# tomneda/DABstar

Hardware: NVIDIA B200
Metric: Mode I DAB frames/s decoded (IQ->Viterbi) (higher is better)
Workload: dtype f32

## Files before the change

### dabstar_b200/csrc/engine.cu

```cuda
#include "../../include/dabstar_b200.h"
#include "kernels.h"
#include "tables.h"
#include "hostpool.h"
#include "fft2048.cuh"

#include <algorithm>
#include <array>
#include <atomic>
#include <chrono>
#include <climits>
#include <cmath>
#include <cstdint>
#include <cstdarg>
#include <cstdio>
#include <cstring>
#include <map>
#include <memory>
#include <string>
#include <vector>

using namespace dab;

namespace
{
// ... 252 lines not shown
  }
  ctx->h_bin_signed.resize(K_CARR);
  host_freq_interleaver(ctx->h_bin_signed.data());
  ctx->h_prs.resize(T_U);
  host_phase_table(ctx->h_prs.data());
  std::vector<float2> w(T_U);
  host_w2048(w.data());
  std::vector<int16_t> bin_idx(K_CARR), rel(K_CARR);
  for (int k = 0; k < K_CARR; k++)
  {
    const int b = ctx->h_bin_signed[k];
    bin_idx[k] = (int16_t)(b < 0 ? b + T_U : b);
    rel[k] = (int16_t)(b < 0 ? b + K_CARR / 2 : b + K_CARR / 2 - 1);
  }
  std::vector<uint8_t> prbs(PRBS_LEN);
  host_prbs(prbs.data(), PRBS_LEN);
  bool ok = true;
  ok = ok && cudaMalloc(&ctx->tab.w2048, sizeof(float2) * T_U) == cudaSuccess;
  ok = ok && cudaMalloc(&ctx->tab.prs, sizeof(float2) * T_U) == cudaSuccess;
  ok = ok && cudaMalloc(&ctx->tab.ref_arg_conj, sizeof(float2) * T_U) == cudaSuccess;
  ok = ok && cudaMalloc(&ctx->tab.bin_of_k, sizeof(int16_t) * K_CARR) == cudaSuccess;
  ok = ok && cudaMalloc(&ctx->tab.rel_of_k, sizeof(int16_t) * K_CARR) == cudaSuccess;
  ok = ok && cudaMalloc(&ctx->tab.prbs, PRBS_LEN) == cudaSuccess;
  std::vector<uint16_t> slot_w(16 * FFT_THREADS), slot_r(K_CARR);
  host_fft_epilogue_layout(bin_idx.data(), slot_w.data(), slot_r.data());
  ok = ok && cudaMalloc(&ctx->tab.fft_slot_w, sizeof(uint16_t) * slot_w.size()) == cudaSuccess;
  ok = ok && cudaMalloc(&ctx->tab.fft_slot_r, sizeof(uint16_t) * slot_r.size()) == cudaSuccess;
  ok = ok && cudaMemcpy(ctx->tab.fft_slot_w, slot_w.data(), sizeof(uint16_t) * slot_w.size(), cudaMemcpyHostToDevice) == cudaSuccess;
  ok = ok && cudaMemcpy(ctx->tab.fft_slot_r, slot_r.data(), sizeof(uint16_t) * slot_r.size(), cudaMemcpyHostToDevice) == cudaSuccess;
  ok = ok && cudaMemcpy(ctx->tab.w2048, w.data(), sizeof(float2) * T_U, cudaMemcpyHostToDevice) == cudaSuccess;
  ok = ok && cudaMemcpy(ctx->tab.prs, ctx->h_prs.data(), sizeof(float2) * T_U, cudaMemcpyHostToDevice) == cudaSuccess;
  ok = ok && cudaMemcpy(ctx->tab.bin_of_k, bin_idx.data(), sizeof(int16_t) * K_CARR, cudaMemcpyHostToDevice) == cudaSuccess;
  ok = ok && cudaMemcpy(ctx->tab.rel_of_k, rel.data(), sizeof(int16_t) * K_CARR, cudaMemcpyHostToDevice) == cudaSuccess;
  ok = ok && cudaMemcpy(ctx->tab.prbs, prbs.data(), PRBS_LEN, cudaMemcpyHostToDevice) == cudaSuccess;
  ok = ok && launch_init_ref_arg(ctx->stream, ctx->tab, &ctx->launches) == cudaSuccess;
  ok = ok && cudaStreamSynchronize(ctx->stream) == cudaSuccess;
  if (!ok) { dabstar_destroy(ctx.release()); return DABSTAR_E_CUDA; }
  push_profile(ctx.get(), make_fic_profile());
  *out = ctx.release();
  return DABSTAR_OK;
}

extern "C" void dabstar_destroy(dabstar_ctx * ctx)
{
  if (!ctx) return;
  cudaSetDevice(ctx->device);
  cudaFree(ctx->tab.w2048); cudaFree(ctx->tab.prs); cudaFree(ctx->tab.ref_arg_conj);
  cudaFree(ctx->tab.bin_of_k); cudaFree(ctx->tab.rel_of_k); cudaFree(ctx->tab.prbs); cudaFree(ctx->tab.fft_slot_w); cudaFree(ctx->tab.fft_slot_r);
// ... 2580 lines not shown
```

### dabstar_b200/csrc/ofdm_kernels.cu

```cuda
#include "fft2048.cuh"
#include "kernels.h"
#include "devcache.h"

#include <algorithm>
#include <cstdlib>
#include <type_traits>

namespace dab
{
namespace
{
template <int FMT> struct Raw;
template <> struct Raw<FMT_U8> { typedef unsigned short type; typedef unsigned reg; };
template <> struct Raw<FMT_I16> { typedef short2 type; typedef short2 reg; };
template <> struct Raw<FMT_CF32> { typedef float2 type; typedef float2 reg; };

__device__ __forceinline__ float2 to_cf(unsigned v)
{
  const float2 m = make_float2(__uint_as_float(__byte_perm(v, 0x4B000000u, 0x7540)), __uint_as_float(__byte_perm(v, 0x4B000000u, 0x7541)));
  const float2 f = __fadd2_rn(m, make_float2(-8388608.0f, -8388608.0f));
  return __ffma2_rn(f, make_float2(1.0f / 128.0f, 1.0f / 128.0f), make_float2(-127.38f / 128.0f, -127.38f / 128.0f));
}
__device__ __forceinline__ float2 to_cf(short2 v) { return __fmul2_rn(make_float2((float)v.x, (float)v.y), make_float2(1.0f / 32768.0f, 1.0f / 32768.0f)); }
__device__ __forceinline__ float2 to_cf(float2 v) { return v; }
// ... 121 lines not shown
__device__ __forceinline__ void bulk_g2s(unsigned dst, const void * src, unsigned bytes, unsigned bar)
{
  asm volatile("cp.async.bulk.shared::cluster.global.mbarrier::complete_tx::bytes [%0], [%1], %2, [%3];" ::"r"(dst), "l"(src), "r"(bytes), "r"(bar) : "memory");
}
__device__ __forceinline__ void mbar_wait(unsigned bar, unsigned parity)
{
  unsigned ok;
  do
  {
    asm volatile("{\n\t.reg .pred p;\n\tmbarrier.try_wait.parity.shared::cta.b64 p, [%1], %2;\n\tselp.u32 %0, 1, 0, p;\n\t}" : "=r"(ok) : "r"(bar), "r"(parity) : "memory");
  } while (!ok);
}

template <int FMT>
__device__ __forceinline__ bool item_async(const SymbolItem & it) { return it.out >= 0 && it.start >= 8 && it.start + T_U + 8 <= it.n_total; }

__device__ __forceinline__ int mod_fs32(int x)
{
  const int r = x % FS;
  return r < 0 ? r + FS : r;
}

template <int FMT>
__device__ __forceinline__ void convert_mix(float2 (&v)[16], const typename Raw<FMT>::reg (&r)[16], int f, int ph, const float2 * step, int tid)
{
#pragma unroll
  for (int n1 = 0; n1 < 16; n1++) v[n1] = to_cf(r[n1]);
  if (f == 0)
  {
    if (ph == 0) return;
    const float2 c = step[0];
#pragma unroll
    for (int n1 = 0; n1 < 16; n1++) v[n1] = cmul(v[n1], c);
    return;
  }
  const float2 s0 = osc(mod_fs32(ph - f * (tid + 1)));
#pragma unroll
  for (int n1 = 0; n1 < 16; n1++) v[n1] = cmul(v[n1], n1 == 0 ? s0 : cmul(s0, step[n1]));
}

template <int FMT>
__global__ void __launch_bounds__(FFT_THREADS, 5) k_fft_frames(const FrameDesc * __restrict__ frames, int n_items, const RecInput * __restrict__ recs,
                                                               const float2 * __restrict__ w2048, const uint16_t * __restrict__ slot_w,
                                                               const uint16_t * __restrict__ slot_r, float2 * __restrict__ X)
{
  typedef typename Raw<FMT>::type T;
  extern __shared__ __align__(16) unsigned char fft_stage[];
  __shared__ __align__(16) float2 smem[FFT_SMEM_F2];
  __shared__ float2 tw2s[FFT_TW2_F2];
  __shared__ float2 step[16];
  __shared__ unsigned short pos[16 * FFT_THREADS];
  __shared__ unsigned rpos[K_CARR / 2];
  __shared__ __align__(8) unsigned long long mbar[2];
  const int tid = threadIdx.x;
  FftTwiddles tw;
  fft_load_twiddles(tw, w2048, tw2s, tid);
#pragma unroll
  for (int i = 0; i < 16; i++) pos[i * FFT_THREADS + tid] = (unsigned short)(slot_w[i * FFT_THREADS + tid] * (int)sizeof(float2));
  for (int p = tid; p < K_CARR / 2; p += FFT_THREADS)
    rpos[p] = (unsigned)slot_r[2 * p] * (unsigned)sizeof(float2) | ((unsigned)slot_r[2 * p + 1] * (unsigned)sizeof(float2)) << 16;
  static_assert(2048 <= FFT_SMEM_F2, "the staging slots (16 per write group) must fit the transform buffer");
  const unsigned stage0 = smem_addr_u32(fft_stage);
  const unsigned bar0 = smem_addr_u32(mbar);
  constexpr int SB = fft_stage_bytes<FMT>();
  if (tid == 0)
  {
    mbar_init(bar0, 1);
    mbar_init(bar0 + 8, 1);
    asm volatile("fence.mbarrier_init.release.cluster;" ::: "memory");
    asm volatile("fence.proxy.async.shared::cta;" ::: "memory");
  }
  __syncthreads();

  const int per = n_items / (int)gridDim.x, rem = n_items - per * (int)gridDim.x;
  int item = (int)blockIdx.x * per + min((int)blockIdx.x, rem);
  const int item_end = item + per + ((int)blockIdx.x < rem ? 1 : 0);
  int buf = 0, fi = item / X_ROWS, row = item - fi * X_ROWS;
  unsigned phase_bits = 0;
  FrameDesc fd;
  RecInput rin;
  SymbolItem cur;
  cur.out = -1;
  int dph = 0;
  int step_f = 0;
  int step_ph = -1;
  auto issue = [&](const SymbolItem & it, int b) {
    if (tid == 0)
    {
      const unsigned long long a = (unsigned long long)(reinterpret_cast<const T *>(it.iq) + it.start);
      mbar_expect_tx(bar0 + 8u * (unsigned)b, (unsigned)SB);
      bulk_g2s(stage0 + (unsigned)(b * SB), reinterpret_cast<const void *>(a & ~15ull), (unsigned)SB, bar0 + 8u * (unsigned)b);
    }
  };
  if (item < item_end)
  {
    fd = frames[fi];
    rin = recs[fd.rec];
    cur = symbol_item(fd, rin, row);
    dph = mod_fs32(-(int)(((long long)fd.f_data * T_S) % FS));
    if (item_async<FMT>(cur)) issue(cur, 0);
  }
  while (item < item_end)
  {
    const int next = item + 1;
    SymbolItem nxt;
    nxt.out = -1;
    if (next < item_end)
    {
      if (++row == X_ROWS)
      {
        row = 0;
        fi++;
        fd = frames[fi];
        rin = recs[fd.rec];
        dph = mod_fs32(-(int)(((long long)fd.f_data * T_S) % FS));
      }
      if (row >= 2 && row <= 75)
      {
        nxt.iq = cur.iq;
        nxt.n_total = cur.n_total;
        nxt.start = cur.start + T_S;
        nxt.f = cur.f;
        nxt.ph = cur.ph + dph;
        if (nxt.ph >= FS) nxt.ph -= FS;
        nxt.out = row > fd.n_syms ? -1 : ((long long)fd.xslot * X_ROWS + row) * K_CARR;
      }
      else nxt = symbol_item(fd, rin, row);
      if (item_async<FMT>(nxt)) issue(nxt, buf ^ 1);
    }
    if (cur.out >= 0)
    {
      float2 v[16];
      if (cur.f != 0 ? cur.f != step_f : (cur.ph != 0 && cur.ph != step_ph))
      {
        __syncthreads();
        if (cur.f != 0)
        {
          if (tid < 16) step[tid] = osc(mod_fs32(-(int)(((long long)cur.f * 128 * tid) % FS)));
          step_f = cur.f;
          step_ph = -1;
        }
        else
        {
          if (tid == 0) step[0] = osc(cur.ph);
          step_ph = cur.ph;
          step_f = 0;
        }
        __syncthreads();
      }
      if (item_async<FMT>(cur))
      {
        mbar_wait(bar0 + 8u * (unsigned)buf, (phase_bits >> buf) & 1u);
        phase_bits ^= 1u << buf;
        const unsigned off = (unsigned)((unsigned long long)(reinterpret_cast<const T *>(cur.iq) + cur.start) & 15ull);
        const T * sp = reinterpret_cast<const T *>(fft_stage + buf * SB + off) + tid;
        typename Raw<FMT>::reg r[16];
#pragma unroll
        for (int n1 = 0; n1 < 16; n1++) r[n1] = sp[128 * n1];
        convert_mix<FMT>(v, r, cur.f, cur.ph, step, tid);
      }
      else
      {
        typename Raw<FMT>::reg r[16];
        fetch_symbol<FMT>(r, cur.iq, cur.n_total, cur.start, tid);
        convert_mix<FMT>(v, r, cur.f, cur.ph, step, tid);
        if (!(cur.start >= 0 && cur.start + T_U <= cur.n_total))
        {
#pragma unroll
          for (int n1 = 0; n1 < 16; n1++)
          {
            const long long i = cur.start + 128 * n1 + tid;
            if (i < 0 || i >= cur.n_total) v[n1] = make_float2(0.0f, 0.0f);
          }
        }
      }
      fft_stage1(v, tw, smem, tid);
      __syncthreads();
      fft_stage2_read(v, smem, tid);
      __syncthreads();
      fft_stage2(v, tw, smem, tid);
      __syncthreads();
      fft_stage3(v, smem, tid);
      __syncthreads();
      unsigned char * sbase = reinterpret_cast<unsigned char *>(smem);
#pragma unroll
      for (int i = 0; i < 16; i++) *reinterpret_cast<float2 *>(sbase + pos[i * FFT_THREADS + tid]) = v[i];
      __syncthreads();
      float4 * out = reinterpret_cast<float4 *>(X + cur.out);
#pragma unroll
      for (int i = 0; i < K_CARR / 2 / FFT_THREADS; i++)
      {
        const int p = tid + FFT_THREADS * i;
        const unsigned rp = rpos[p];
        const float2 a = *reinterpret_cast<const float2 *>(sbase + (rp & 0xffffu)), b = *reinterpret_cast<const float2 *>(sbase + (rp >> 16));
        out[p] = make_float4(a.x, b.x, a.y, b.y);
      }
    }
    __syncthreads();
    cur = nxt;
    item = next;
    buf ^= 1;
  }
}

__global__ void __launch_bounds__(FFT_THREADS, 4) k_fft_batch(const float2 * __restrict__ in, float2 * __restrict__ out, int n, int sign,
                                                              const float2 * __restrict__ w2048)
{
  __shared__ float2 smem[FFT_SMEM_F2];
  __shared__ float2 tw2s[FFT_TW2_F2];
  const int tid = threadIdx.x;
  FftTwiddles tw;
  fft_load_twiddles(tw, w2048, tw2s, tid);
  __syncthreads();
  for (int item = blockIdx.x; item < n; item += gridDim.x)
  {
    float2 v[16];
#pragma unroll
    for (int n1 = 0; n1 < 16; n1++)
    {
      v[n1] = in[(size_t)item * T_U + 128 * n1 + tid];
      if (sign > 0) v[n1].y = -v[n1].y;
    }
    fft2048_to_smem(v, tw, smem, tid);
    for (int i = tid; i < T_U; i += FFT_THREADS)
    {
      float2 r = smem[fft_nat(i)];
      if (sign > 0) r.y = -r.y;
      out[(size_t)item * T_U + i] = r;
    }
    __syncthreads();
  }
}

template <int FMT>
__global__ void __launch_bounds__(FFT_THREADS, 4) k_fft_null(const FrameDesc * __restrict__ frames, int n_frames, const RecInput * __restrict__ recs,
                                                             const float2 * __restrict__ w2048, float2 * __restrict__ out)
{
  __shared__ float2 smem[FFT_SMEM_F2];
  __shared__ float2 step[16];
  __shared__ float2 tw2s[FFT_TW2_F2];
  const int tid = threadIdx.x;
  FftTwiddles tw;
  fft_load_twiddles(tw, w2048, tw2s, tid);
  __syncthreads();
  for (int fi = blockIdx.x; fi < n_frames; fi += gridDim.x)
  {
    const FrameDesc fd = frames[fi];
    const RecInput rin = recs[fd.rec];
    const SymbolItem it = symbol_item(fd, rin, X_ROWS - 1);
    float2 v[16];
    load_symbol<FMT>(v, it.iq, it.n_total, it.start, it.f, it.ph, step, tid);
    if (!(it.start >= 0 && it.start + T_U <= it.n_total))
    {
#pragma unroll
      for (int n1 = 0; n1 < 16; n1++)
      {
        const long long i = it.start + 128 * n1 + tid;
        if (i < 0 || i >= it.n_total) v[n1] = make_float2(0.0f, 0.0f);
      }
    }
    fft2048_to_smem(v, tw, smem, tid);
    for (int i = tid; i < T_U; i += FFT_THREADS) out[(size_t)fi * T_U + i] = smem[fft_nat(i)];
    __syncthreads();
  }
}

__global__ void k_reorder_frames(const float2 * __restrict__ fft_nat, int n_rows, const int16_t * __restrict__ bin_of_k, float2 * __restrict__ X)
{
  const int row = blockIdx.x;
  if (row >= n_rows) return;
  for (int p = threadIdx.x; p < K_CARR / 2; p += blockDim.x)
  {
    const float2 a = fft_nat[(size_t)row * T_U + bin_of_k[2 * p]], b = fft_nat[(size_t)row * T_U + bin_of_k[2 * p + 1]];
    reinterpret_cast<float4 *>(X + (size_t)row * K_CARR)[p] = make_float4(a.x, b.x, a.y, b.y);
  }
}

__device__ __forceinline__ float warp_sum(float v)
{
#pragma unroll
  for (int o = 16; o > 0; o >>= 1) v += __shfl_xor_sync(0xffffffffu, v, o);
  return v;
}

__device__ void prs_correlate_cta(float2 (&v)[16], const FftTwiddles & tw, const float2 * __restrict__ prs, float threshold, int strongest,
                                  float2 * smem, float * red, int * result, int tid)
// ... 1067 lines not shown
    const long long b = o >> 11;
    const int j = (int)(o & 2047);
    const long long lo = b * block_in + base[j] - shift;
    const float r = frac[j], r1 = __fsub_rn(1.0f, r);
    const float2 hi_v = lo + 1 < n_in ? in[lo + 1] : make_float2(0.f, 0.f);
    const float2 lo_v = lo >= 0 ? in[lo] : make_float2(0.f, 0.f);
    out[o] = make_float2(__fadd_rn(__fmul_rn(hi_v.x, r), __fmul_rn(lo_v.x, r1)), __fadd_rn(__fmul_rn(hi_v.y, r), __fmul_rn(lo_v.y, r1)));
  }
}

template <typename F> cudaError_t dispatch_fmt(int fmt, F && f)
{
  switch (fmt)
  {
  case FMT_CF32: f(std::integral_constant<int, FMT_CF32>()); break;
  case FMT_U8: f(std::integral_constant<int, FMT_U8>()); break;
  case FMT_I16: f(std::integral_constant<int, FMT_I16>()); break;
  default: return cudaErrorInvalidValue;
  }
  return cudaGetLastError();
}

inline int fft_grid(int n_items) { return n_items < N_SM * 4 ? n_items : N_SM * 4; }
}

cudaError_t launch_init_ref_arg(cudaStream_t s, const DeviceTables & t, unsigned long long * lc)
{
  k_init_ref_arg<<<1, FFT_THREADS, 0, s>>>(t.w2048, t.prs, t.ref_arg_conj);
  if (lc) (*lc)++;
  return cudaGetLastError();
}

cudaError_t launch_fft_batch(cudaStream_t s, const DeviceTables & t, const float2 * in, float2 * out, int n, int sign, unsigned long long * lc)
{
  if (n <= 0) return cudaSuccess;
  k_fft_batch<<<fft_grid(n), FFT_THREADS, 0, s>>>(in, out, n, sign, t.w2048);
  if (lc) (*lc)++;
  return cudaGetLastError();
}

cudaError_t launch_fft_frames(cudaStream_t s, const DeviceTables & t, const FrameDesc * frames, int n_frames, const RecInput * recs, int fmt,
                              float2 * X, int max_ctas_per_sm, unsigned long long * lc)
{
  if (n_frames <= 0) return cudaSuccess;
  const int n_items = n_frames * X_ROWS;
  if (lc) (*lc)++;
  return dispatch_fmt(fmt, [&](auto F) {
    constexpr int FMT = decltype(F)::value;
    constexpr int stage = 2 * fft_stage_bytes<FMT>();
    const LaunchProps lp = launch_props((const void *)k_fft_frames<FMT>, FFT_THREADS, stage, stage);
    int per_sm = lp.err == cudaSuccess && lp.ctas_per_sm > 0 ? lp.ctas_per_sm : 4;
    if (max_ctas_per_sm > 0) per_sm = std::min(per_sm, max_ctas_per_sm);
    k_fft_frames<FMT><<<std::min(n_items, lp.n_sm * per_sm), FFT_THREADS, stage, s>>>(frames, n_items, recs, t.w2048, t.fft_slot_w, t.fft_slot_r, X);
  });
}

cudaError_t launch_reorder_frames(cudaStream_t s, const DeviceTables & t, const float2 * fft_nat, int n_frames, float2 * X, unsigned long long * lc)
{
  if (n_frames <= 0) return cudaSuccess;
  k_reorder_frames<<<n_frames * X_ROWS, 256, 0, s>>>(fft_nat, n_frames * X_ROWS, t.bin_of_k, X);
  if (lc) (*lc)++;
  return cudaGetLastError();
}

size_t demap_ring_bytes(int n_work) { return sizeof(unsigned long long) * (size_t)std::max(n_work, 1) * DM3_RING * DM5_WARPS + 256; }
static size_t demap5_smem_bytes(int lag) { return sizeof(float4) * 2 * (size_t)(lag + 1 + DM5_PF) * DM5_T + sizeof(int) * (size_t)(lag + 1) * (DM5_T / 32); }
template <int LAG, bool QUAL> static const void * demap5_fn(int soft_bit_type)
{
  return soft_bit_type == 0 ? (const void *)k_demap5<0, LAG, QUAL> : (soft_bit_type == 1 ? (const void *)k_demap5<1, LAG, QUAL> : (const void *)k_demap5<2, LAG, QUAL>);
}
template <int LAG> static const void * demap5_fn(int soft_bit_type, bool qual) { return qual ? demap5_fn<LAG, true>(soft_bit_type) : demap5_fn<LAG, false>(soft_bit_type); }

cudaError_t launch_demap(cudaStream_t s, const DeviceTables & t, const DemapWork * work, int n_work, const FrameDesc * frames,
                         const uint8_t * null_is_tii, const float2 * X, OfdmStateDev * states, int soft_bit_type, int16_t * soft,
                         unsigned long long * ring, FrameQualSnap * qsnap, unsigned long long * lc)
{
// ... 97 lines not shown
{
  if (n <= 0) return cudaSuccess;
  k_coarse_afc_raw<<<fft_grid(n), FFT_THREADS, 0, s>>>(fft_nat, n, t.w2048, t.ref_arg_conj, offset_hz);
  if (lc) (*lc)++;
  return cudaGetLastError();
}

cudaError_t launch_ingest_convert(cudaStream_t s, const void * src, int container, int msb_first, int iq_order, float inv_scaler, const float * lut,
                                  long long n_samples, float2 * dst, unsigned long long * lc)
{
  if (n_samples <= 0) return cudaSuccess;
  const long long blocks = (n_samples + 255) / 256;
  k_ingest_convert<<<(unsigned)std::min<long long>(blocks, N_SM * 16), 256, 0, s>>>(static_cast<const unsigned char *>(src), container, msb_first, iq_order, inv_scaler, lut,
                                                                                    n_samples, dst);
  if (lc) (*lc)++;
  return cudaGetLastError();
}

cudaError_t launch_fft_null(cudaStream_t s, const DeviceTables & t, const FrameDesc * frames, int n_frames, const RecInput * recs, int fmt, float2 * out,
                            unsigned long long * lc)
{
  if (n_frames <= 0) return cudaSuccess;
  if (lc) (*lc)++;
  return dispatch_fmt(fmt, [&](auto F) { k_fft_null<decltype(F)::value><<<fft_grid(n_frames), FFT_THREADS, 0, s>>>(frames, n_frames, recs, t.w2048, out); });
}

cudaError_t launch_resample_linear(cudaStream_t s, const float2 * in, long long n_in, int block_in, int shift, const short * base, const float * frac,
                                   long long n_out, float2 * out, unsigned long long * lc)
{
  if (n_out <= 0) return cudaSuccess;
  const long long blocks = (n_out + 255) / 256;
  k_resample_linear<<<(unsigned)std::min<long long>(blocks, N_SM * 16), 256, 0, s>>>(in, n_in, block_in, shift, base, frac, n_out, out);
  if (lc) (*lc)++;
  return cudaGetLastError();
}

cudaError_t launch_dip_search(cudaStream_t s, const DipWork * work, int n, const RecInput * recs, int fmt, DipResult * out, unsigned long long * lc)
{
  if (n <= 0) return cudaSuccess;
  if (lc) (*lc)++;
  return dispatch_fmt(fmt, [&](auto F) { k_dip_search<decltype(F)::value><<<n, DIP_THREADS, 0, s>>>(work, recs, out); });
}
}
```

### dabstar_b200/csrc/tables.cu

```cuda
#include "tables.h"
#include "fft2048.cuh"
#include <vector>

#include <cmath>
#include <cstring>

namespace dab
{
static const uint32_t PI_MASK[24] = {
  0x11111113u, 0x11131113u, 0x11131313u, 0x13131313u, 0x13131333u, 0x13331333u, 0x13333333u, 0x33333333u,
  0x33333337u, 0x33373337u, 0x33373737u, 0x37373737u, 0x37373777u, 0x37773777u, 0x37777777u, 0x77777777u,
  0x7777777fu, 0x777f777fu, 0x777f7f7fu, 0x7f7f7f7fu, 0x7f7f7fffu, 0x7fff7fffu, 0x7fffffffu, 0xffffffffu };

struct UepRow { int16_t bitrate, level, L[4], PI[4]; };
static const UepRow UEP_TABLE[] = {
  {32,5, {3,4,17,0}, {5,3,2,0}}, {32,4, {3,3,18,0}, {11,6,5,0}}, {32,3, {3,4,14,3}, {15,9,6,8}},
  {32,2, {3,4,14,3}, {22,13,8,13}}, {32,1, {3,5,13,3}, {24,17,12,17}}, {48,5, {4,3,26,3}, {5,4,2,3}},
  {48,4, {3,4,26,3}, {9,6,4,6}}, {48,3, {3,4,26,3}, {15,10,6,9}}, {48,2, {3,4,26,3}, {24,14,8,15}},
  {48,1, {3,5,25,3}, {24,18,13,18}}, {56,5, {6,10,23,3}, {5,4,2,3}}, {56,4, {6,10,23,3}, {9,6,4,5}},
  {56,3, {6,12,21,3}, {16,7,6,9}}, {56,2, {6,10,23,3}, {23,13,8,13}}, {64,5, {6,9,31,2}, {5,3,2,3}},
  {64,4, {6,9,33,0}, {11,6,5,0}}, {64,3, {6,12,27,3}, {16,8,6,9}}, {64,2, {6,10,29,3}, {23,13,8,13}},
  {64,1, {6,11,28,3}, {24,18,12,18}}, {80,5, {6,10,41,3}, {6,3,2,3}}, {80,4, {6,10,41,3}, {11,6,5,6}},
  {80,3, {6,11,40,3}, {16,8,6,7}}, {80,2, {6,10,41,3}, {23,13,8,13}}, {80,1, {6,10,41,3}, {24,7,12,18}},
  {96,5, {7,9,53,3}, {5,4,2,4}}, {96,4, {7,10,52,3}, {9,6,4,6}}, {96,3, {6,12,51,3}, {16,9,6,10}},
// ... 13 lines not shown
static const int N_UEP = (int)(sizeof(UEP_TABLE) / sizeof(UEP_TABLE[0]));

static const uint8_t PRS_ROW[48] = { 0,1,2,3, 0,1,2,3, 0,1,2,3, 0,1,2,3, 0,1,2,3, 0,1,2,3,
                                     0,3,2,1, 0,3,2,1, 0,3,2,1, 0,3,2,1, 0,3,2,1, 0,3,2,1 };
static const uint8_t PRS_N[48] = { 1,2,0,1, 3,2,2,3, 2,1,2,3, 1,2,3,3, 2,2,2,1, 1,3,1,2,
                                   3,1,1,1, 2,2,1,0, 2,2,3,3, 0,2,1,3, 3,3,3,0, 3,0,1,1 };
static const uint8_t PRS_H[4][32] = {
  { 0,2,0,0,0,0,1,1,2,0,0,0,2,2,1,1, 0,2,0,0,0,0,1,1,2,0,0,0,2,2,1,1 },
  { 0,3,2,3,0,1,3,0,2,1,2,3,2,3,3,0, 0,3,2,3,0,1,3,0,2,1,2,3,2,3,3,0 },
  { 0,0,0,2,0,2,1,3,2,2,0,2,2,0,1,3, 0,0,0,2,0,2,1,3,2,2,0,2,2,0,1,3 },
  { 0,1,2,1,0,3,3,2,2,3,2,1,2,1,3,2, 0,1,2,1,0,3,3,2,2,3,2,1,2,1,3,2 } };

void host_freq_interleaver(int16_t * bin_signed)
{
  int n = 0, v = 0;
  for (int i = 0; i < T_U; i++)
  {
    if (i > 0) v = (13 * v + 511) % T_U;
    if (v == T_U / 2 || v < 256 || v > 256 + K_CARR) continue;
    bin_signed[n++] = (int16_t)(v - T_U / 2);
  }
}

void host_fft_epilogue_layout(const int16_t * bin_of_k, uint16_t * slot_w, uint16_t * slot_r)
{
  constexpr int NW = 128, NR = 96, D = 16;
  std::vector<int> carrier_of_bin(T_U, -1);
  for (int k = 0; k < K_CARR; k++) carrier_of_bin[bin_of_k[k]] = k;
  std::vector<int> wg(K_CARR, -1), rg(K_CARR, -1);
  for (int i = 0; i < 16; i++)
    for (int tid = 0; tid < FFT_THREADS; tid++)
    {
      const int c = carrier_of_bin[fft_out_index(tid, i >> 3, i & 7)];
      if (c >= 0) wg[c] = (i * 4 + (tid >> 5)) * 2 + ((tid >> 4) & 1);
    }
  for (int c = 0; c < K_CARR; c++)
  {
    const int p = c >> 1, b = c & 1, it = p / FFT_THREADS, tid = p % FFT_THREADS;
    rg[c] = ((it * 2 + b) * 4 + (tid >> 5)) * 2 + ((tid >> 4) & 1);
  }
  std::vector<int> at_w(NW * D, -1), at_r(NR * D, -1), colour(K_CARR, -1);
  for (int e = 0; e < K_CARR; e++)
  {
    const int u = wg[e], v = rg[e];
    int a = 0, b = 0;
    while (at_w[u * D + a] >= 0) a++;
    while (at_r[v * D + b] >= 0) b++;
    if (a != b)
    {
      std::vector<int> path;
      int x = v, side = 1, want = a;
      while (true)
      {
        const int f = side ? at_r[x * D + want] : at_w[x * D + want];
        if (f < 0) break;
        path.push_back(f);
        x = side ? wg[f] : rg[f];
        side ^= 1;
        want = want == a ? b : a;
      }
      for (int f : path) { at_w[wg[f] * D + colour[f]] = -1; at_r[rg[f] * D + colour[f]] = -1; }
      for (int f : path) { colour[f] = colour[f] == a ? b : a; }
      for (int f : path) { at_w[wg[f] * D + colour[f]] = f; at_r[rg[f] * D + colour[f]] = f; }
    }
    colour[e] = a;
    at_w[u * D + a] = e;
    at_r[v * D + a] = e;
  }
  for (int c = 0; c < K_CARR; c++) slot_r[c] = (uint16_t)(wg[c] * D + colour[c]);
  for (int i = 0; i < 16; i++)
    for (int tid = 0; tid < FFT_THREADS; tid++)
    {
      const int g = (i * 4 + (tid >> 5)) * 2 + ((tid >> 4) & 1);
      const int c = carrier_of_bin[fft_out_index(tid, i >> 3, i & 7)];
      if (c >= 0) { slot_w[i * FFT_THREADS + tid] = slot_r[c]; continue; }
      int a = 0;
      while (at_w[g * D + a] >= 0) a++;
      at_w[g * D + a] = K_CARR;
      slot_w[i * FFT_THREADS + tid] = (uint16_t)(g * D + a);
    }
}

void host_phase_table(float2 * prs)
{
  const float pi_2 = (float)(M_PI / 2.0);
  memset(prs, 0, sizeof(float2) * T_U);
  for (int k = -K_CARR / 2; k <= K_CARR / 2; k++)
  {
    if (k == 0) continue;
    const int blk = k < 0 ? (k + 768) / 32 : 24 + (k - 1) / 32;
    const int kmin = k < 0 ? -768 + 32 * blk : 1 + 32 * (blk - 24);
    const float phi = pi_2 * (float)(PRS_H[PRS_ROW[blk]][k - kmin] + PRS_N[blk]);
    prs[k < 0 ? k + T_U : k] = make_float2(cosf(phi), sinf(phi));
  }
}

void host_prbs(uint8_t * out, int n)
{
  unsigned reg = 0x1ff;
  for (int i = 0; i < n; i++)
  {
    const unsigned b = ((reg >> 8) ^ (reg >> 4)) & 1u;
    reg = ((reg << 1) | b) & 0x1ff;
// ... 111 lines not shown
```

### dabstar_b200/csrc/tables.h

```cpp
#pragma once
#include "common.cuh"
#include "viterbi.cuh"

namespace dab
{
void host_freq_interleaver(int16_t * bin_signed);
void host_phase_table(float2 * prs);
void host_prbs(uint8_t * out, int n);
void host_w2048(float2 * w);
void host_fft_epilogue_layout(const int16_t * bin_of_k, uint16_t * slot_w , uint16_t * slot_r );
VitProfile make_fic_profile();
VitProfile make_identity_profile(int n_bits);
bool make_msc_profile(int short_form, int bit_rate, int prot_level, VitProfile & p);
int profile_addresses(const VitProfile & p, int32_t * addr, int cap);
}
```

Before: 792,800.

## Move 2048-point FFT to one warp per symbol with warp-local epilogue

Replaces the 128-thread block-cooperative 2048-point FFT with a per-warp FFT: each lane holds 64 points, runs a radix-64 then radix-32 decomposition with a single padded shared-memory transpose, and synchronises with __syncwarp instead of __syncthreads. Work is split across warps with per-warp TMA staging buffers and mbarriers, and the bank-conflict-free carrier scatter layout is recomputed for the warp output order. The aim is to remove block-wide barriers and improve independent progress per warp. In exchange it adds heavy register pressure (64 complex values per thread plus raw inputs), uses more shared memory per warp, and runs one CTA per SM, which may lower occupancy.

```diff
diff --git a/dabstar_b200/csrc/engine.cu b/dabstar_b200/csrc/engine.cu
--- a/dabstar_b200/csrc/engine.cu
+++ b/dabstar_b200/csrc/engine.cu
@@ -298,8 +298,8 @@
   ok = ok && cudaMalloc(&ctx->tab.bin_of_k, sizeof(int16_t) * K_CARR) == cudaSuccess;
   ok = ok && cudaMalloc(&ctx->tab.rel_of_k, sizeof(int16_t) * K_CARR) == cudaSuccess;
   ok = ok && cudaMalloc(&ctx->tab.prbs, PRBS_LEN) == cudaSuccess;
-  std::vector<uint16_t> slot_w(16 * FFT_THREADS), slot_r(K_CARR);
-  host_fft_epilogue_layout(bin_idx.data(), slot_w.data(), slot_r.data());
+  std::vector<uint16_t> slot_w(T_U), slot_r(K_CARR);
+  host_fft_warp_epilogue_layout(bin_idx.data(), slot_w.data(), slot_r.data());
   ok = ok && cudaMalloc(&ctx->tab.fft_slot_w, sizeof(uint16_t) * slot_w.size()) == cudaSuccess;
   ok = ok && cudaMalloc(&ctx->tab.fft_slot_r, sizeof(uint16_t) * slot_r.size()) == cudaSuccess;
   ok = ok && cudaMemcpy(ctx->tab.fft_slot_w, slot_w.data(), sizeof(uint16_t) * slot_w.size(), cudaMemcpyHostToDevice) == cudaSuccess;
diff --git a/dabstar_b200/csrc/fft2048_warp.cuh b/dabstar_b200/csrc/fft2048_warp.cuh
--- /dev/null
+++ b/dabstar_b200/csrc/fft2048_warp.cuh
@@ -0,0 +1,134 @@
+#pragma once
+#include "fft2048.cuh"
+
+namespace dab
+{
+constexpr int FFTW_E_STRIDE = 33;
+constexpr int FFTW_E_F2 = 64 * FFTW_E_STRIDE;
+constexpr int FFTW_TW_F2 = 64 * 32;
+
+__host__ __device__ inline void fftw_load_twiddles(const float2 * w2048, float2 * tw, int tid, int nthreads)
+{
+  for (int i = tid; i < FFTW_TW_F2; i += nthreads) tw[i] = w2048[((i & 31) * (i >> 5)) & 2047];
+}
+
+__host__ __device__ constexpr float cos64(int r)
+{
+  switch (r)
+  {
+  case 0: return 1.0f;
+  case 1: return 0.99518472667219688624f;
+  case 2: return 0.98078528040323044913f;
+  case 3: return 0.95694033573220886494f;
+  case 4: return 0.92387953251128675613f;
+  case 5: return 0.88192126434835502971f;
+  case 6: return 0.83146961230254523708f;
+  case 7: return 0.77301045336273696081f;
+  case 8: return 0.70710678118654752440f;
+  case 9: return 0.63439328416364549822f;
+  case 10: return 0.55557023301960222474f;
+  case 11: return 0.47139673682599764856f;
+  case 12: return 0.38268343236508977173f;
+  case 13: return 0.29028467725446236764f;
+  case 14: return 0.19509032201612826785f;
+  case 15: return 0.09801714032956060199f;
+  default: return 0.0f;
+  }
+}
+
+__host__ __device__ __forceinline__ float2 mul_w64(float2 a, int e)
+{
+  e &= 63;
+  if (e == 0) return a;
+  if (e == 16) return cmul_mj(a);
+  const int q = e >> 4, r = e & 15;
+  const float c = cos64(r), s = cos64(16 - r);
+  switch (q)
+  {
+  case 0: return cmul_const(a, c, -s);
+  case 1: return cmul_const(a, -s, -c);
+  case 2: return cmul_const(a, -c, s);
+  default: return cmul_const(a, s, c);
+  }
+}
+
+template <int S> __host__ __device__ __forceinline__ void dft8s(float2 * v)
+{
+  float2 t[8];
+#pragma unroll
+  for (int i = 0; i < 8; i++) t[i] = v[S * i];
+  dft8(t);
+#pragma unroll
+  for (int i = 0; i < 8; i++) v[S * i] = t[i];
+}
+
+__host__ __device__ __forceinline__ void dft64(float2 (&v)[64])
+{
+#pragma unroll
+  for (int b = 0; b < 8; b++) dft8s<8>(&v[b]);
+#pragma unroll
+  for (int c = 1; c < 8; c++)
+#pragma unroll
+    for (int b = 1; b < 8; b++) v[8 * c + b] = mul_w64(v[8 * c + b], b * c);
+#pragma unroll
+  for (int c = 0; c < 8; c++) dft8s<1>(&v[8 * c]);
+#pragma unroll
+  for (int c = 0; c < 8; c++)
+#pragma unroll
+    for (int d = c + 1; d < 8; d++)
+    {
+      const float2 t = v[8 * c + d];
+      v[8 * c + d] = v[8 * d + c];
+      v[8 * d + c] = t;
+    }
+}
+
+__host__ __device__ __forceinline__ void dft32(float2 * v)
+{
+#pragma unroll
+  for (int b = 0; b < 4; b++) dft8s<4>(&v[b]);
+#pragma unroll
+  for (int c = 1; c < 8; c++)
+#pragma unroll
+    for (int b = 1; b < 4; b++) v[4 * c + b] = mul_w64(v[4 * c + b], 2 * b * c);
+#pragma unroll
+  for (int c = 0; c < 8; c++) dft4(v[4 * c], v[4 * c + 1], v[4 * c + 2], v[4 * c + 3]);
+  float2 t[32];
+#pragma unroll
+  for (int c = 0; c < 8; c++)
+#pragma unroll
+    for (int d = 0; d < 4; d++) t[c + 8 * d] = v[4 * c + d];
+#pragma unroll
+  for (int i = 0; i < 32; i++) v[i] = t[i];
+}
+
+__host__ __device__ __forceinline__ void fftw_stage1(float2 (&v)[64], const float2 * tw, float2 * e, int lane)
+{
+  dft64(v);
+#pragma unroll
+  for (int k1 = 0; k1 < 64; k1++) e[k1 * FFTW_E_STRIDE + lane] = k1 == 0 ? v[0] : cmul(v[k1], tw[k1 * 32 + lane]);
+}
+
+__host__ __device__ __forceinline__ void fftw_stage2(float2 (&v)[64], const float2 * e, int lane)
+{
+#pragma unroll
+  for (int h = 0; h < 2; h++)
+  {
+#pragma unroll
+    for (int l = 0; l < 32; l++) v[32 * h + l] = e[(lane + 32 * h) * FFTW_E_STRIDE + l];
+    dft32(&v[32 * h]);
+  }
+}
+
+__host__ __device__ inline int fftw_out_index(int lane, int i) { return lane + 32 * (i >> 5) + 64 * (i & 31); }
+
+#ifdef __CUDACC__
+__device__ __forceinline__ void fft2048_warp(float2 (&v)[64], const float2 * tw, float2 * e, int lane)
+{
+  fftw_stage1(v, tw, e, lane);
+  __syncwarp();
+  fftw_stage2(v, e, lane);
+  __syncwarp();
+}
+#endif
+}
diff --git a/dabstar_b200/csrc/ofdm_kernels.cu b/dabstar_b200/csrc/ofdm_kernels.cu
--- a/dabstar_b200/csrc/ofdm_kernels.cu
+++ b/dabstar_b200/csrc/ofdm_kernels.cu
@@ -1,4 +1,4 @@
-#include "fft2048.cuh"
+#include "fft2048_warp.cuh"
 #include "kernels.h"
 #include "devcache.h"
 
@@ -167,48 +167,105 @@
 }
 
 template <int FMT>
-__device__ __forceinline__ void convert_mix(float2 (&v)[16], const typename Raw<FMT>::reg (&r)[16], int f, int ph, const float2 * step, int tid)
-{
-#pragma unroll
-  for (int n1 = 0; n1 < 16; n1++) v[n1] = to_cf(r[n1]);
+__device__ __forceinline__ void fetch_symbol_w(typename Raw<FMT>::reg (&r)[64], const void * __restrict__ iq, long long n_total, long long start, int lane)
+{
+  typedef typename Raw<FMT>::type T;
+  const T * p = reinterpret_cast<const T *>(iq) + start + lane;
+  if (start >= 0 && start + T_U <= n_total)
+  {
+#pragma unroll
+    for (int m = 0; m < 64; m++) r[m] = p[32 * m];
+  }
+  else
+  {
+#pragma unroll
+    for (int m = 0; m < 64; m++)
+    {
+      const long long i = start + 32 * m + lane;
+      if (i >= 0 && i < n_total) r[m] = p[32 * m];
+      else r[m] = typename Raw<FMT>::reg();
+    }
+  }
+}
+
+__device__ __forceinline__ void fill_step_w(float2 * step, int f, int ph, int lane)
+{
+  if (f != 0)
+  {
+#pragma unroll
+    for (int h = 0; h < 2; h++) step[lane + 32 * h] = osc(mod_fs32(-(int)(((long long)f * 32 * (lane + 32 * h)) % FS)));
+  }
+  else if (lane == 0) step[0] = osc(ph);
+}
+
+template <int FMT>
+__device__ __forceinline__ void convert_mix_w(float2 (&v)[64], const typename Raw<FMT>::reg (&r)[64], int f, int ph, const float2 * step, int lane)
+{
+#pragma unroll
+  for (int m = 0; m < 64; m++) v[m] = to_cf(r[m]);
   if (f == 0)
   {
     if (ph == 0) return;
     const float2 c = step[0];
 #pragma unroll
-    for (int n1 = 0; n1 < 16; n1++) v[n1] = cmul(v[n1], c);
+    for (int m = 0; m < 64; m++) v[m] = cmul(v[m], c);
     return;
   }
-  const float2 s0 = osc(mod_fs32(ph - f * (tid + 1)));
-#pragma unroll
-  for (int n1 = 0; n1 < 16; n1++) v[n1] = cmul(v[n1], n1 == 0 ? s0 : cmul(s0, step[n1]));
-}
+  const float2 s0 = osc(mod_fs32(ph - f * (lane + 1)));
+#pragma unroll
+  for (int m = 0; m < 64; m++) v[m] = cmul(v[m], m == 0 ? s0 : cmul(s0, step[m]));
+}
+
+__device__ __forceinline__ void zero_outside_w(float2 (&v)[64], long long n_total, long long start, int lane)
+{
+  if (start >= 0 && start + T_U <= n_total) return;
+#pragma unroll
+  for (int m = 0; m < 64; m++)
+  {
+    const long long i = start + 32 * m + lane;
+    if (i < 0 || i >= n_total) v[m] = make_float2(0.0f, 0.0f);
+  }
+}
+
+template <int FMT> struct FftWarpShape
+{
+  static constexpr int SB = fft_stage_bytes<FMT>();
+  static constexpr int PER_WARP = FFTW_E_F2 * (int)sizeof(float2) + 2 * SB + 64 * (int)sizeof(float2) + 16;
+  static constexpr int WARPS = FMT == FMT_U8 ? 8 : FMT == FMT_I16 ? 6 : 4;
+  static constexpr int DYN = WARPS * PER_WARP;
+  static_assert(PER_WARP % 16 == 0 && SB % 16 == 0, "TMA destinations must stay 16-byte aligned");
+};
 
 template <int FMT>
-__global__ void __launch_bounds__(FFT_THREADS, 5) k_fft_frames(const FrameDesc * __restrict__ frames, int n_items, const RecInput * __restrict__ recs,
-                                                               const float2 * __restrict__ w2048, const uint16_t * __restrict__ slot_w,
-                                                               const uint16_t * __restrict__ slot_r, float2 * __restrict__ X)
-{
+__global__ void __launch_bounds__(FftWarpShape<FMT>::WARPS * 32, 1)
+k_fft_frames(const FrameDesc * __restrict__ frames, int n_items, const RecInput * __restrict__ recs, const float2 * __restrict__ w2048,
+             const uint16_t * __restrict__ slot_w, const uint16_t * __restrict__ slot_r, float2 * __restrict__ X)
+{
+  typedef FftWarpShape<FMT> S;
   typedef typename Raw<FMT>::type T;
-  extern __shared__ __align__(16) unsigned char fft_stage[];
-  __shared__ __align__(16) float2 smem[FFT_SMEM_F2];
-  __shared__ float2 tw2s[FFT_TW2_F2];
-  __shared__ float2 step[16];
-  __shared__ unsigned short pos[16 * FFT_THREADS];
+  extern __shared__ __align__(16) unsigned char fft_dyn[];
+  __shared__ __align__(16) float2 tw[FFTW_TW_F2];
+  __shared__ unsigned wcol[16 * 32];
   __shared__ unsigned rpos[K_CARR / 2];
-  __shared__ __align__(8) unsigned long long mbar[2];
-  const int tid = threadIdx.x;
-  FftTwiddles tw;
-  fft_load_twiddles(tw, w2048, tw2s, tid);
-#pragma unroll
-  for (int i = 0; i < 16; i++) pos[i * FFT_THREADS + tid] = (unsigned short)(slot_w[i * FFT_THREADS + tid] * (int)sizeof(float2));
-  for (int p = tid; p < K_CARR / 2; p += FFT_THREADS)
+  const int tid = threadIdx.x, lane = tid & 31, warp = tid >> 5;
+  fftw_load_twiddles(w2048, tw, tid, S::WARPS * 32);
+  for (int j = tid; j < 16 * 32; j += S::WARPS * 32)
+  {
+    const int q = j >> 5, l = j & 31;
+    unsigned w = 0;
+#pragma unroll
+    for (int b = 0; b < 4; b++) w |= (unsigned)(slot_w[(4 * q + b) * 32 + l] & 15) * (unsigned)sizeof(float2) << (8 * b);
+    wcol[j] = w;
+  }
+  for (int p = tid; p < K_CARR / 2; p += S::WARPS * 32)
     rpos[p] = (unsigned)slot_r[2 * p] * (unsigned)sizeof(float2) | ((unsigned)slot_r[2 * p + 1] * (unsigned)sizeof(float2)) << 16;
-  static_assert(2048 <= FFT_SMEM_F2, "the staging slots (16 per write group) must fit the transform buffer");
-  const unsigned stage0 = smem_addr_u32(fft_stage);
-  const unsigned bar0 = smem_addr_u32(mbar);
-  constexpr int SB = fft_stage_bytes<FMT>();
-  if (tid == 0)
+  unsigned char * wbase = fft_dyn + warp * S::PER_WARP;
+  float2 * e = reinterpret_cast<float2 *>(wbase);
+  unsigned char * stage = wbase + FFTW_E_F2 * sizeof(float2);
+  float2 * step = reinterpret_cast<float2 *>(stage + 2 * S::SB);
+  const unsigned stage0 = smem_addr_u32(stage);
+  const unsigned bar0 = smem_addr_u32(step + 64);
+  if (lane == 0)
   {
     mbar_init(bar0, 1);
     mbar_init(bar0 + 8, 1);
@@ -217,9 +274,10 @@
   }
   __syncthreads();
 
-  const int per = n_items / (int)gridDim.x, rem = n_items - per * (int)gridDim.x;
-  int item = (int)blockIdx.x * per + min((int)blockIdx.x, rem);
-  const int item_end = item + per + ((int)blockIdx.x < rem ? 1 : 0);
+  const int n_warps = (int)gridDim.x * S::WARPS, gw = (int)blockIdx.x * S::WARPS + warp;
+  const int per = n_items / n_warps, rem = n_items - per * n_warps;
+  int item = gw * per + min(gw, rem);
+  const int item_end = item + per + (gw < rem ? 1 : 0);
   int buf = 0, fi = item / X_ROWS, row = item - fi * X_ROWS;
   unsigned phase_bits = 0;
   FrameDesc fd;
@@ -230,11 +288,11 @@
   int step_f = 0;
   int step_ph = -1;
   auto issue = [&](const SymbolItem & it, int b) {
-    if (tid == 0)
+    if (lane == 0)
     {
       const unsigned long long a = (unsigned long long)(reinterpret_cast<const T *>(it.iq) + it.start);
-      mbar_expect_tx(bar0 + 8u * (unsigned)b, (unsigned)SB);
-      bulk_g2s(stage0 + (unsigned)(b * SB), reinterpret_cast<const void *>(a & ~15ull), (unsigned)SB, bar0 + 8u * (unsigned)b);
+      mbar_expect_tx(bar0 + 8u * (unsigned)b, (unsigned)S::SB);
+      bulk_g2s(stage0 + (unsigned)(b * S::SB), reinterpret_cast<const void *>(a & ~15ull), (unsigned)S::SB, bar0 + 8u * (unsigned)b);
     }
   };
   if (item < item_end)
@@ -275,138 +333,120 @@
     }
     if (cur.out >= 0)
     {
-      float2 v[16];
       if (cur.f != 0 ? cur.f != step_f : (cur.ph != 0 && cur.ph != step_ph))
       {
-        __syncthreads();
-        if (cur.f != 0)
-        {
-          if (tid < 16) step[tid] = osc(mod_fs32(-(int)(((long long)cur.f * 128 * tid) % FS)));
-          step_f = cur.f;
-          step_ph = -1;
-        }
-        else
-        {
-          if (tid == 0) step[0] = osc(cur.ph);
-          step_ph = cur.ph;
-          step_f = 0;
-        }
-        __syncthreads();
+        __syncwarp();
+        fill_step_w(step, cur.f, cur.ph, lane);
+        step_f = cur.f;
+        step_ph = cur.f != 0 ? -1 : cur.ph;
+        __syncwarp();
       }
+      float2 v[64];
+      typename Raw<FMT>::reg r[64];
       if (item_async<FMT>(cur))
       {
         mbar_wait(bar0 + 8u * (unsigned)buf, (phase_bits >> buf) & 1u);
         phase_bits ^= 1u << buf;
         const unsigned off = (unsigned)((unsigned long long)(reinterpret_cast<const T *>(cur.iq) + cur.start) & 15ull);
-        const T * sp = reinterpret_cast<const T *>(fft_stage + buf * SB + off) + tid;
-        typename Raw<FMT>::reg r[16];
-#pragma unroll
-        for (int n1 = 0; n1 < 16; n1++) r[n1] = sp[128 * n1];
-        convert_mix<FMT>(v, r, cur.f, cur.ph, step, tid);
+        const T * sp = reinterpret_cast<const T *>(stage + buf * S::SB + off) + lane;
+#pragma unroll
+        for (int m = 0; m < 64; m++) r[m] = sp[32 * m];
+        convert_mix_w<FMT>(v, r, cur.f, cur.ph, step, lane);
       }
       else
       {
-        typename Raw<FMT>::reg r[16];
-        fetch_symbol<FMT>(r, cur.iq, cur.n_total, cur.start, tid);
-        convert_mix<FMT>(v, r, cur.f, cur.ph, step, tid);
-        if (!(cur.start >= 0 && cur.start + T_U <= cur.n_total))
-        {
-#pragma unroll
-          for (int n1 = 0; n1 < 16; n1++)
-          {
-            const long long i = cur.start + 128 * n1 + tid;
-            if (i < 0 || i >= cur.n_total) v[n1] = make_float2(0.0f, 0.0f);
-          }
-        }
+        fetch_symbol_w<FMT>(r, cur.iq, cur.n_total, cur.start, lane);
+        convert_mix_w<FMT>(v, r, cur.f, cur.ph, step, lane);
+        zero_outside_w(v, cur.n_total, cur.start, lane);
       }
-      fft_stage1(v, tw, smem, tid);
-      __syncthreads();
-      fft_stage2_read(v, smem, tid);
-      __syncthreads();
-      fft_stage2(v, tw, smem, tid);
-      __syncthreads();
-      fft_stage3(v, smem, tid);
-      __syncthreads();
-      unsigned char * sbase = reinterpret_cast<unsigned char *>(smem);
-#pragma unroll
-      for (int i = 0; i < 16; i++) *reinterpret_cast<float2 *>(sbase + pos[i * FFT_THREADS + tid]) = v[i];
-      __syncthreads();
+      fft2048_warp(v, tw, e, lane);
+      unsigned char * wslot = reinterpret_cast<unsigned char *>(e) + sizeof(float2) * (lane & 16);
+#pragma unroll
+      for (int q = 0; q < 16; q++)
+      {
+        const unsigned w = wcol[q * 32 + lane];
+#pragma unroll
+        for (int b = 0; b < 4; b++)
+          *reinterpret_cast<float2 *>(wslot + 32 * sizeof(float2) * (4 * q + b) + __byte_perm(w, 0u, 0x4440u + b)) = v[4 * q + b];
+      }
+      __syncwarp();
+      const unsigned char * sbase = reinterpret_cast<const unsigned char *>(e);
       float4 * out = reinterpret_cast<float4 *>(X + cur.out);
 #pragma unroll
-      for (int i = 0; i < K_CARR / 2 / FFT_THREADS; i++)
+      for (int i = 0; i < K_CARR / 2 / 32; i++)
       {
-        const int p = tid + FFT_THREADS * i;
+        const int p = lane + 32 * i;
         const unsigned rp = rpos[p];
         const float2 a = *reinterpret_cast<const float2 *>(sbase + (rp & 0xffffu)), b = *reinterpret_cast<const float2 *>(sbase + (rp >> 16));
         out[p] = make_float4(a.x, b.x, a.y, b.y);
       }
     }
-    __syncthreads();
+    __syncwarp();
     cur = nxt;
     item = next;
     buf ^= 1;
   }
 }
 
-__global__ void __launch_bounds__(FFT_THREADS, 4) k_fft_batch(const float2 * __restrict__ in, float2 * __restrict__ out, int n, int sign,
-                                                              const float2 * __restrict__ w2048)
-{
-  __shared__ float2 smem[FFT_SMEM_F2];
-  __shared__ float2 tw2s[FFT_TW2_F2];
-  const int tid = threadIdx.x;
-  FftTwiddles tw;
-  fft_load_twiddles(tw, w2048, tw2s, tid);
-  __syncthreads();
-  for (int item = blockIdx.x; item < n; item += gridDim.x)
-  {
-    float2 v[16];
-#pragma unroll
-    for (int n1 = 0; n1 < 16; n1++)
-    {
-      v[n1] = in[(size_t)item * T_U + 128 * n1 + tid];
-      if (sign > 0) v[n1].y = -v[n1].y;
-    }
-    fft2048_to_smem(v, tw, smem, tid);
-    for (int i = tid; i < T_U; i += FFT_THREADS)
-    {
-      float2 r = smem[fft_nat(i)];
+constexpr int FFTW_TAP_WARPS = 4;
+constexpr int FFTW_TAP_DYN = FFTW_TAP_WARPS * FFTW_E_F2 * (int)sizeof(float2) + FFTW_TAP_WARPS * 64 * (int)sizeof(float2);
+
+__global__ void __launch_bounds__(FFTW_TAP_WARPS * 32) k_fft_batch(const float2 * __restrict__ in, float2 * __restrict__ out, int n, int sign,
+                                                                 const float2 * __restrict__ w2048)
+{
+  extern __shared__ __align__(16) unsigned char fft_dyn[];
+  __shared__ __align__(16) float2 tw[FFTW_TW_F2];
+  const int tid = threadIdx.x, lane = tid & 31, warp = tid >> 5;
+  float2 * e = reinterpret_cast<float2 *>(fft_dyn) + warp * FFTW_E_F2;
+  fftw_load_twiddles(w2048, tw, tid, FFTW_TAP_WARPS * 32);
+  __syncthreads();
+  for (int item = blockIdx.x * FFTW_TAP_WARPS + warp; item < n; item += gridDim.x * FFTW_TAP_WARPS)
+  {
+    float2 v[64];
+#pragma unroll
+    for (int m = 0; m < 64; m++)
+    {
+      v[m] = in[(size_t)item * T_U + 32 * m + lane];
+      if (sign > 0) v[m].y = -v[m].y;
+    }
+    fft2048_warp(v, tw, e, lane);
+#pragma unroll
+    for (int i = 0; i < 64; i++)
+    {
+      float2 r = v[i];
       if (sign > 0) r.y = -r.y;
-      out[(size_t)item * T_U + i] = r;
-    }
-    __syncthreads();
+      out[(size_t)item * T_U + fftw_out_index(lane, i)] = r;
+    }
   }
 }
 
 template <int FMT>
-__global__ void __launch_bounds__(FFT_THREADS, 4) k_fft_null(const FrameDesc * __restrict__ frames, int n_frames, const RecInput * __restrict__ recs,
-                                                             const float2 * __restrict__ w2048, float2 * __restrict__ out)
-{
-  __shared__ float2 smem[FFT_SMEM_F2];
-  __shared__ float2 step[16];
-  __shared__ float2 tw2s[FFT_TW2_F2];
-  const int tid = threadIdx.x;
-  FftTwiddles tw;
-  fft_load_twiddles(tw, w2048, tw2s, tid);
-  __syncthreads();
-  for (int fi = blockIdx.x; fi < n_frames; fi += gridDim.x)
+__global__ void __launch_bounds__(FFTW_TAP_WARPS * 32) k_fft_null(const FrameDesc * __restrict__ frames, int n_frames, const RecInput * __restrict__ recs,
+                                                                const float2 * __restrict__ w2048, float2 * __restrict__ out)
+{
+  extern __shared__ __align__(16) unsigned char fft_dyn[];
+  __shared__ __align__(16) float2 tw[FFTW_TW_F2];
+  const int tid = threadIdx.x, lane = tid & 31, warp = tid >> 5;
+  float2 * e = reinterpret_cast<float2 *>(fft_dyn) + warp * FFTW_E_F2;
+  float2 * step = reinterpret_cast<float2 *>(fft_dyn) + FFTW_TAP_WARPS * FFTW_E_F2 + warp * 64;
+  fftw_load_twiddles(w2048, tw, tid, FFTW_TAP_WARPS * 32);
+  __syncthreads();
+  for (int fi = blockIdx.x * FFTW_TAP_WARPS + warp; fi < n_frames; fi += gridDim.x * FFTW_TAP_WARPS)
   {
     const FrameDesc fd = frames[fi];
     const RecInput rin = recs[fd.rec];
     const SymbolItem it = symbol_item(fd, rin, X_ROWS - 1);
-    float2 v[16];
-    load_symbol<FMT>(v, it.iq, it.n_total, it.start, it.f, it.ph, step, tid);
-    if (!(it.start >= 0 && it.start + T_U <= it.n_total))
-    {
-#pragma unroll
-      for (int n1 = 0; n1 < 16; n1++)
-      {
-        const long long i = it.start + 128 * n1 + tid;
-        if (i < 0 || i >= it.n_total) v[n1] = make_float2(0.0f, 0.0f);
-      }
-    }
-    fft2048_to_smem(v, tw, smem, tid);
-    for (int i = tid; i < T_U; i += FFT_THREADS) out[(size_t)fi * T_U + i] = smem[fft_nat(i)];
-    __syncthreads();
+    typename Raw<FMT>::reg r[64];
+    fetch_symbol_w<FMT>(r, it.iq, it.n_total, it.start, lane);
+    __syncwarp();
+    fill_step_w(step, it.f, it.ph, lane);
+    __syncwarp();
+    float2 v[64];
+    convert_mix_w<FMT>(v, r, it.f, it.ph, step, lane);
+    zero_outside_w(v, it.n_total, it.start, lane);
+    fft2048_warp(v, tw, e, lane);
+#pragma unroll
+    for (int i = 0; i < 64; i++) out[(size_t)fi * T_U + fftw_out_index(lane, i)] = v[i];
   }
 }
 
@@ -1520,6 +1560,11 @@
 }
 
 inline int fft_grid(int n_items) { return n_items < N_SM * 4 ? n_items : N_SM * 4; }
+inline int fftw_tap_grid(int n_items, const LaunchProps & lp)
+{
+  const int per_sm = lp.ctas_per_sm > 0 ? lp.ctas_per_sm : 1;
+  return std::min((n_items + FFTW_TAP_WARPS - 1) / FFTW_TAP_WARPS, std::max(lp.n_sm, 1) * per_sm);
+}
 }
 
 cudaError_t launch_init_ref_arg(cudaStream_t s, const DeviceTables & t, unsigned long long * lc)
@@ -1532,7 +1577,9 @@
 cudaError_t launch_fft_batch(cudaStream_t s, const DeviceTables & t, const float2 * in, float2 * out, int n, int sign, unsigned long long * lc)
 {
   if (n <= 0) return cudaSuccess;
-  k_fft_batch<<<fft_grid(n), FFT_THREADS, 0, s>>>(in, out, n, sign, t.w2048);
+  const LaunchProps lp = launch_props((const void *)k_fft_batch, FFTW_TAP_WARPS * 32, FFTW_TAP_DYN, FFTW_TAP_DYN);
+  if (lp.err != cudaSuccess) return lp.err;
+  k_fft_batch<<<fftw_tap_grid(n, lp), FFTW_TAP_WARPS * 32, FFTW_TAP_DYN, s>>>(in, out, n, sign, t.w2048);
   if (lc) (*lc)++;
   return cudaGetLastError();
 }
@@ -1545,11 +1592,12 @@
   if (lc) (*lc)++;
   return dispatch_fmt(fmt, [&](auto F) {
     constexpr int FMT = decltype(F)::value;
-    constexpr int stage = 2 * fft_stage_bytes<FMT>();
-    const LaunchProps lp = launch_props((const void *)k_fft_frames<FMT>, FFT_THREADS, stage, stage);
-    int per_sm = lp.err == cudaSuccess && lp.ctas_per_sm > 0 ? lp.ctas_per_sm : 4;
+    typedef FftWarpShape<FMT> S;
+    const LaunchProps lp = launch_props((const void *)k_fft_frames<FMT>, S::WARPS * 32, S::DYN, S::DYN);
+    int per_sm = lp.err == cudaSuccess && lp.ctas_per_sm > 0 ? lp.ctas_per_sm : 1;
     if (max_ctas_per_sm > 0) per_sm = std::min(per_sm, max_ctas_per_sm);
-    k_fft_frames<FMT><<<std::min(n_items, lp.n_sm * per_sm), FFT_THREADS, stage, s>>>(frames, n_items, recs, t.w2048, t.fft_slot_w, t.fft_slot_r, X);
+    const int ctas = std::min((n_items + S::WARPS - 1) / S::WARPS, lp.n_sm * per_sm);
+    k_fft_frames<FMT><<<ctas, S::WARPS * 32, S::DYN, s>>>(frames, n_items, recs, t.w2048, t.fft_slot_w, t.fft_slot_r, X);
   });
 }
 
@@ -1693,7 +1741,10 @@
 {
   if (n_frames <= 0) return cudaSuccess;
   if (lc) (*lc)++;
-  return dispatch_fmt(fmt, [&](auto F) { k_fft_null<decltype(F)::value><<<fft_grid(n_frames), FFT_THREADS, 0, s>>>(frames, n_frames, recs, t.w2048, out); });
+  return dispatch_fmt(fmt, [&](auto F) {
+    const LaunchProps lp = launch_props((const void *)k_fft_null<decltype(F)::value>, FFTW_TAP_WARPS * 32, FFTW_TAP_DYN, FFTW_TAP_DYN);
+    k_fft_null<decltype(F)::value><<<fftw_tap_grid(n_frames, lp), FFTW_TAP_WARPS * 32, FFTW_TAP_DYN, s>>>(frames, n_frames, recs, t.w2048, out);
+  });
 }
 
 cudaError_t launch_resample_linear(cudaStream_t s, const float2 * in, long long n_in, int block_in, int shift, const short * base, const float * frac,
diff --git a/dabstar_b200/csrc/tables.cu b/dabstar_b200/csrc/tables.cu
--- a/dabstar_b200/csrc/tables.cu
+++ b/dabstar_b200/csrc/tables.cu
@@ -1,5 +1,5 @@
 #include "tables.h"
-#include "fft2048.cuh"
+#include "fft2048_warp.cuh"
 #include <vector>
 
 #include <cmath>
@@ -59,24 +59,19 @@
   }
 }
 
-void host_fft_epilogue_layout(const int16_t * bin_of_k, uint16_t * slot_w, uint16_t * slot_r)
-{
-  constexpr int NW = 128, NR = 96, D = 16;
+static void colour_epilogue(const int16_t * bin_of_k, const int * bin_of_value, const int * wg_of_value, const int * rg_of_carrier, int n_rg,
+                            uint16_t * slot_w, uint16_t * slot_r)
+{
+  constexpr int NW = T_U / 16, D = 16;
   std::vector<int> carrier_of_bin(T_U, -1);
   for (int k = 0; k < K_CARR; k++) carrier_of_bin[bin_of_k[k]] = k;
-  std::vector<int> wg(K_CARR, -1), rg(K_CARR, -1);
-  for (int i = 0; i < 16; i++)
-    for (int tid = 0; tid < FFT_THREADS; tid++)
-    {
-      const int c = carrier_of_bin[fft_out_index(tid, i >> 3, i & 7)];
-      if (c >= 0) wg[c] = (i * 4 + (tid >> 5)) * 2 + ((tid >> 4) & 1);
-    }
-  for (int c = 0; c < K_CARR; c++)
-  {
-    const int p = c >> 1, b = c & 1, it = p / FFT_THREADS, tid = p % FFT_THREADS;
-    rg[c] = ((it * 2 + b) * 4 + (tid >> 5)) * 2 + ((tid >> 4) & 1);
-  }
-  std::vector<int> at_w(NW * D, -1), at_r(NR * D, -1), colour(K_CARR, -1);
+  std::vector<int> wg(K_CARR, -1), rg(rg_of_carrier, rg_of_carrier + K_CARR);
+  for (int v = 0; v < T_U; v++)
+  {
+    const int c = carrier_of_bin[bin_of_value[v]];
+    if (c >= 0) wg[c] = wg_of_value[v];
+  }
+  std::vector<int> at_w(NW * D, -1), at_r(n_rg * D, -1), colour(K_CARR, -1);
   for (int e = 0; e < K_CARR; e++)
   {
     const int u = wg[e], v = rg[e];
@@ -105,17 +100,50 @@
     at_r[v * D + a] = e;
   }
   for (int c = 0; c < K_CARR; c++) slot_r[c] = (uint16_t)(wg[c] * D + colour[c]);
+  for (int v = 0; v < T_U; v++)
+  {
+    const int g = wg_of_value[v];
+    const int c = carrier_of_bin[bin_of_value[v]];
+    if (c >= 0) { slot_w[v] = slot_r[c]; continue; }
+    int a = 0;
+    while (at_w[g * D + a] >= 0) a++;
+    at_w[g * D + a] = K_CARR;
+    slot_w[v] = (uint16_t)(g * D + a);
+  }
+}
+
+void host_fft_epilogue_layout(const int16_t * bin_of_k, uint16_t * slot_w, uint16_t * slot_r)
+{
+  std::vector<int> bin(T_U), wg(T_U), rg(K_CARR);
   for (int i = 0; i < 16; i++)
     for (int tid = 0; tid < FFT_THREADS; tid++)
     {
-      const int g = (i * 4 + (tid >> 5)) * 2 + ((tid >> 4) & 1);
-      const int c = carrier_of_bin[fft_out_index(tid, i >> 3, i & 7)];
-      if (c >= 0) { slot_w[i * FFT_THREADS + tid] = slot_r[c]; continue; }
-      int a = 0;
-      while (at_w[g * D + a] >= 0) a++;
-      at_w[g * D + a] = K_CARR;
-      slot_w[i * FFT_THREADS + tid] = (uint16_t)(g * D + a);
-    }
+      bin[i * FFT_THREADS + tid] = fft_out_index(tid, i >> 3, i & 7);
+      wg[i * FFT_THREADS + tid] = (i * 4 + (tid >> 5)) * 2 + ((tid >> 4) & 1);
+    }
+  for (int c = 0; c < K_CARR; c++)
+  {
+    const int p = c >> 1, b = c & 1, it = p / FFT_THREADS, tid = p % FFT_THREADS;
+    rg[c] = ((it * 2 + b) * 4 + (tid >> 5)) * 2 + ((tid >> 4) & 1);
+  }
+  colour_epilogue(bin_of_k, bin.data(), wg.data(), rg.data(), 96, slot_w, slot_r);
+}
+
+void host_fft_warp_epilogue_layout(const int16_t * bin_of_k, uint16_t * slot_w, uint16_t * slot_r)
+{
+  std::vector<int> bin(T_U), wg(T_U), rg(K_CARR);
+  for (int i = 0; i < 64; i++)
+    for (int l = 0; l < 32; l++)
+    {
+      bin[i * 32 + l] = fftw_out_index(l, i);
+      wg[i * 32 + l] = 2 * i + (l >> 4);
+    }
+  for (int c = 0; c < K_CARR; c++)
+  {
+    const int p = c >> 1, b = c & 1, it = p / 32, l = p % 32;
+    rg[c] = (it * 2 + b) * 2 + (l >> 4);
+  }
+  colour_epilogue(bin_of_k, bin.data(), wg.data(), rg.data(), K_CARR / 16, slot_w, slot_r);
 }
 
 void host_phase_table(float2 * prs)
diff --git a/dabstar_b200/csrc/tables.h b/dabstar_b200/csrc/tables.h
--- a/dabstar_b200/csrc/tables.h
+++ b/dabstar_b200/csrc/tables.h
@@ -9,6 +9,7 @@
 void host_prbs(uint8_t * out, int n);
 void host_w2048(float2 * w);
 void host_fft_epilogue_layout(const int16_t * bin_of_k, uint16_t * slot_w , uint16_t * slot_r );
+void host_fft_warp_epilogue_layout(const int16_t * bin_of_k, uint16_t * slot_w , uint16_t * slot_r );
 VitProfile make_fic_profile();
 VitProfile make_identity_profile(int n_bits);
 bool make_msc_profile(int short_form, int bit_rate, int prot_level, VitProfile & p);
```

Result: no change. 781,600, median of 6 (-1.4%).
